# flanggut/smvs

Hardware: NVIDIA H100
Metric: Gauss-Newton Mpix-iters/sec (higher is better)
Workload: dtype f64

## Files before the change

smvs_b200/csrc/api.cu:

```cuda
#include <algorithm>
#include <atomic>
#include <cmath>
#include <cstring>
#include <dlfcn.h>

#include "common.cuh"

namespace smvsb {
void fill_basis_table (std::vector<double>& tab, int ps, int step);
void device_set_scale (smvsb_ctx* c, uint8_t const* img_dev, int w, int h,
    int scale, float* tmp_a, float* tmp_b, int mode, float* out_dev);
void device_shading_inputs (smvsb_ctx* c, uint8_t const* img_dev, int w, int h,
    float* shading_dev, float* shading_grad_dev);
void device_set_scale_float (smvsb_ctx* c, float const* img_dev, int w, int h,
    int scale, float* tmp_a, float* tmp_b, float* out_dev);
void device_set_scale_rgb (smvsb_ctx* c, float const* img_dev, int w, int h,
    int scale, float* tmp_a, float* tmp_b, int mode, float* out_dev,
    float* blur_out);
void device_bilateral_filter (smvsb_ctx* c, float const* ci_dev, int w, int h,
    int channels, float const* dm_dev, int dm_w, int dm_h, float sigma,
    int kernel_size, float* out_dev);
float host_expf_like_glibc (float x);
void device_byte_to_float (smvsb_ctx* c, uint8_t const* img_dev, size_t n,
    float* out_dev);
// ... 176 lines not shown
                    V[i * N + q] = sn * vp + cs * vq;
                }
            }
        if (off < 1e-15)
            break;
    }
    double sinv[16];
    for (int j = 0; j < N; ++j)
    {
        double n = 0.0;
        for (int i = 0; i < N; ++i) n += U[i * N + j] * U[i * N + j];
        n = std::sqrt(n);
        for (int i = 0; i < N; ++i)
            U[i * N + j] = (n > 0.0 ? U[i * N + j] / n : 0.0);
        sinv[j] = (n >= -1e-12 && n <= 1e-12) ? 0.0 : 1.0 / n;
    }
    for (int i = 0; i < N; ++i)
        for (int j = 0; j < N; ++j)
        {
            double s = 0.0;
            for (int k = 0; k < N; ++k)
                s += V[i * N + k] * sinv[k] * U[j * N + k];
            Ainv[i * N + j] = s;
        }
}

void
ensure_system_buffers (smvsb_ctx* c)
{
    size_t const np = c->n_patches, nn = c->n_nodes;
    c->patch_H.reserve(np * 256);
    c->patch_g.reserve(np * 16);
    c->patch_proc.reserve(np);
    c->H.reserve(nn * 144);
    c->P.reserve(nn * 16);
    c->g.reserve(nn * 4);
    c->x.reserve(nn * 4);
    c->light.reserve(16);
}

void
set_active (smvsb_ctx* c, uint8_t const* active_nodes)
{
    if (active_nodes != nullptr)
        upload(c, c->active, active_nodes, c->n_nodes);
    else
    {
        c->active.reserve(c->n_nodes);
        CUDA_CHECK(cudaMemcpyAsync(c->active.p, c->node_valid.p, c->n_nodes,
            cudaMemcpyDeviceToDevice, c->stream));
    }
}

void
construct (smvsb_ctx* c, double const* light16, double reg, double light_reg)
{
    require(c->have_views && c->have_surface, SMVSB_ERR_STATE,
        "smvsb_set_views and smvsb_set_surface must precede construct");
    if (light16 != nullptr)
    {
        require(c->have_shading, SMVSB_ERR_STATE,
            "lighting given but the main view has no shading image");
        upload(c, c->light, light16, 16);
    }
    ensure_system_buffers(c);
    smvsb::launch_construct(c, light16 != nullptr, reg, light_reg);
// ... 1557 lines not shown
```

smvs_b200/csrc/common.cuh:

```cuda
#ifndef SMVSB_COMMON_CUH
#define SMVSB_COMMON_CUH

#include <cuda_runtime.h>

#include <atomic>
#include <cstdint>
#include <cstdio>
#include <string>
#include <vector>

#include "../../include/smvs_b200.h"

#define SMVSB_MAX_SUBS 32
#define SMVSB_NB_STRIDE 8
#define SMVSB_NUM_EVENTS 6

#define CUDA_CHECK(call)                                                     \
    do {                                                                     \
        cudaError_t e__ = (call);                                            \
        if (e__ != cudaSuccess)                                              \
            throw smvsb::Error(SMVSB_ERR_CUDA, std::string(#call) + ": "     \
                + cudaGetErrorString(e__));                                  \
    } while (0)

// ... 83 lines not shown
    smvsb::DevBuf<float> main_grad, main_shading, main_shading_grad;
    bool have_shading = false;
    smvsb::SubViewDev subs[SMVSB_MAX_SUBS];
    smvsb::DevBuf<float const*> sub_ptrs;
    smvsb::DevBuf<int> sub_dims;
    smvsb::DevBuf<double> Mt;
    smvsb::DevBuf<uint8_t> stage_u8;
    smvsb::DevBuf<uint8_t> stage_u8b;
    smvsb::DevBuf<float> stage_a, stage_b;
    smvsb::DevBuf<float> view_in, view_texels, view_out;

    bool have_surface = false;
    int scale = 0, ps = 0, sampling = 0, npos = 0;
    int npx = 0, npy = 0, start_x = 0, start_y = 0;
    int n_nodes = 0, n_patches = 0;
    smvsb::DevBuf<double> nodes;
    smvsb::DevBuf<uint8_t> node_valid, patch_valid, vis_ids;
    smvsb::DevBuf<uint32_t> vis_off;
    smvsb::DevBuf<uint8_t> active, active_new;
    smvsb::DevBuf<double> basis_s, basis_f;
    std::vector<uint8_t> h_node_valid, h_patch_valid;

    smvsb::DevBuf<float> init_depth;
    smvsb::DevBuf<double> nodes_tmp;
    smvsb::DevBuf<uint8_t> node_valid_tmp;
    smvsb::DevBuf<uint8_t> u8_main;
    smvsb::DevBuf<uint8_t> u8_subs[SMVSB_MAX_SUBS];
    smvsb::DevBuf<float> guide;

    bool have_system = false;
    smvsb::DevBuf<double> patch_H;
    smvsb::DevBuf<double> patch_g;
    smvsb::DevBuf<uint8_t> patch_proc;
    smvsb::DevBuf<double> H;
    smvsb::DevBuf<double> P;
    smvsb::DevBuf<double> g;
    smvsb::DevBuf<double> light;

    smvsb::DevBuf<double> x, r, d, d2, z, Ad;
    size_t x_count = 0;
    smvsb::DevBuf<double> cg_partials;
    smvsb::DevBuf<uint16_t> cg_rowmask;
    smvsb::DevBuf<uint32_t> cg_row_list, cg_block_rows;
    smvsb::DevBuf<unsigned long long> cg_counts;
    uint64_t cg_blocks = 0, cg_rows = 0;
    double* h_scalars = nullptr;
    smvsb::DevBuf<unsigned int> cg_sync;
    smvsb::DevBuf<double> cg_result;

    smvsb::DevBuf<double> patch_shift;
    smvsb::DevBuf<double> upd_partials, upd_result;
    smvsb::DevBuf<unsigned long long> counters;

    smvsb::DevBuf<unsigned int> zbuf, vis_mask;
    smvsb::DevBuf<unsigned long long> zoff;
    smvsb::DevBuf<float> sgm_depth;
    bool have_color = false;
    smvsb::DevBuf<float> color_main;
    smvsb::DevBuf<float> color_subs[SMVSB_MAX_SUBS];
    smvsb::DevBuf<float const*> color_ptrs;
    smvsb::DevBuf<short4> rim_lists;
    int rim_ps = 0;
    int rim_off[9] = {};
    smvsb::DevBuf<uint32_t> vis_counts;

    smvsb::DevBuf<double> light_partials;
// ... 87 lines not shown
```

smvs_b200/csrc/gn_construct.cu:

```cuda
#include "gn_math.cuh"
#include "patch_eval.cuh"

namespace smvsb {

namespace {

constexpr int K1_THREADS = 128;
constexpr int AS_STRIDE = 27;

__host__ __device__ inline void
hermite (double t, double* b0, double* b1, double* b2)
{
    double const t2 = t * t, t3 = t2 * t;
    b0[0] = 2 * t3 - 3 * t2 + 1;
    b0[1] = -2 * t3 + 3 * t2;
    b0[2] = t3 - 2 * t2 + t;
    b0[3] = t3 - t2;
    b1[0] = 6 * t2 - 6 * t;
    b1[1] = -6 * t2 + 6 * t;
    b1[2] = 3 * t2 - 4 * t + 1;
    b1[3] = 3 * t2 - 2 * t;
    b2[0] = 12 * t - 6;
    b2[1] = -12 * t + 6;
    b2[2] = 6 * t - 4;
    b2[3] = 6 * t - 2;
}

}

void
fill_basis_table (std::vector<double>& tab, int ps, int step)
{
    int const npos = ps / step;
    tab.assign(3 * npos * 4, 0.0);
    for (int a = 0; a < npos; ++a)
    {
        double b0[4], b1[4], b2[4];
        hermite((a * step + 0.5) / ps, b0, b1, b2);
        for (int i = 0; i < 4; ++i)
        {
            tab[(0 * npos + a) * 4 + i] = b0[i];
// ... 9 lines not shown
    float const* __restrict__ hess, float* __restrict__ texels, int n)
{
    int i = blockIdx.x * blockDim.x + threadIdx.x;
    if (i >= n)
        return;
    float4 a, b;
    a.x = grad[2 * i]; a.y = grad[2 * i + 1];
    a.z = hess[3 * i]; a.w = hess[3 * i + 1];
    b.x = hess[3 * i + 2]; b.y = 0.f; b.z = 0.f; b.w = 0.f;
    reinterpret_cast<float4*>(texels)[2 * i] = a;
    reinterpret_cast<float4*>(texels)[2 * i + 1] = b;
}

void
launch_pack_subview (smvsb_ctx* c, float const* grad, float const* hess,
    float* texels, int w, int h)
{
    int const n = w * h;
    pack_subview_kernel<<<(n + 255) / 256, 256, 0, c->stream>>>(grad, hess,
        texels, n);
    smvsb::count_launches(c, 1);
    CUDA_CHECK(cudaGetLastError());
}


struct ConstructArgs
{
    SurfaceDev s;
    double regularization;
    double light_surf_regularization;
    double const* light;
    double* patch_H;
    double* patch_g;
    uint8_t* patch_proc;
};

template <int S, int MINB = 4>
__global__ void __launch_bounds__(K1_THREADS, MINB)
gn_patch_kernel (ConstructArgs const args)
{
    constexpr int SPC = (S < K1_THREADS) ? S : K1_THREADS;
    constexpr int CHUNKS = S / SPC;
    constexpr int PPB = (S >= 16) ? K1_THREADS / SPC : 8;
    constexpr int GSZ = (S >= 16) ? 16 : S;
    constexpr int GPP = (S >= 16) ? SPC / 16 : 1;
    SurfaceDev const& sf = args.s;

    __shared__ double s_theta[PPB][16];
    __shared__ double s_coef[PPB][16];
    __shared__ double s_as[K1_THREADS * AS_STRIDE];
    __shared__ double s_basis[3 * 16 * 4];
    __shared__ double s_part[(GPP > 1) ? K1_THREADS * 17 : 1];
    __shared__ int s_proc[PPB];

    int const tid = threadIdx.x;
    int const npos = sf.npos;

    for (int i = tid; i < 3 * npos * 4; i += K1_THREADS)
        s_basis[i] = sf.basis_s[i];

    if (tid < PPB)
    {
        int const patch = blockIdx.x * PPB + tid;
        int proc = 0;
        if (patch < sf.n_patches && sf.patch_valid[patch])
        {
            int const idx = patch % sf.npx, idy = patch / sf.npx;
            int const n0 = idy * (sf.npx + 1) + idx;
            proc = sf.active[n0] | sf.active[n0 + 1]
                | sf.active[n0 + sf.npx + 1] | sf.active[n0 + sf.npx + 2];
            proc = proc != 0;
        }
        s_proc[tid] = proc;
        if (patch < sf.n_patches)
            args.patch_proc[patch] = static_cast<uint8_t>(proc);
    }
    if (tid < PPB * 16)
    {
        int const pl = tid / 16, col = tid % 16;
        int const patch = blockIdx.x * PPB + pl;
        double v = 0.0;
        if (patch < sf.n_patches)
        {
            int const idx = patch % sf.npx, idy = patch / sf.npx;
            int const node = (idy + ((col >> 3) & 1)) * (sf.npx + 1)
                + idx + ((col >> 2) & 1);
            v = sf.nodes[node * 4 + (col & 3)];
        }
        s_theta[pl][col] = v;
    }
    __syncthreads();

    if (tid < PPB * 16)
    {
        int const pl = tid / 16, r = tid % 16;
        xd sum(0.0);
#pragma unroll
        for (int k = 0; k < 16; ++k)
        {
            double const xv = s_theta[pl][(k & 3) * 4 + (k >> 2)];
            sum += xd(c_hermite[r * 16 + k]) * xd(xv);
        }
        s_coef[pl][(r & 3) * 4 + (r >> 2)] = sum.v;
    }
    __syncthreads();

    int const q = tid / 16;
    int const row = tid % 16;
    int const pl2 = q / GPP;
    int const patch2 = blockIdx.x * PPB + pl2;
    bool const proc2 = s_proc[pl2] != 0;
    double hrow[16];
    double grow = 0.0;
#pragma unroll
    for (int i = 0; i < 16; ++i) hrow[i] = 0.0;

    for (int chunk = 0; chunk < CHUNKS; ++chunk)
    {
    if (tid < PPB * SPC)
    {
        int const pl = tid / SPC;
        int const s = chunk * SPC + tid % SPC;
        int const patch = blockIdx.x * PPB + pl;
        double A[21], b[6];
#pragma unroll
        for (int i = 0; i < 21; ++i) A[i] = 0.0;
#pragma unroll
        for (int i = 0; i < 6; ++i) b[i] = 0.0;

        if (s_proc[pl])
        {
            int const ix = s % npos, iy = s / npos;

            double w, wx, wy, wxy, wxx, wyy;
            {
                double const* cf = s_coef[pl];
                xd const inv_size(1.0 / static_cast<double>(sf.ps));
                xd const sx = (xd(static_cast<double>(ix * sf.sampling))
                    + xd(0.5)) * inv_size;
                xd const sy = (xd(static_cast<double>(iy * sf.sampling))
                    + xd(0.5)) * inv_size;
                xd ex[4], ey[4];
                ex[0] = xd(1.0); ex[1] = sx; ex[2] = sx * sx; ex[3] = ex[2] * sx;
                ey[0] = xd(1.0); ey[1] = sy; ey[2] = sy * sy; ey[3] = ey[2] * sy;
                xd f(0.0), fx(0.0), fy(0.0), fxy(0.0), fxx(0.0), fyy(0.0);
#pragma unroll
                for (int i = 0; i < 4; ++i)
#pragma unroll
                    for (int j = 0; j < 4; ++j)
                        f += xd(cf[i * 4 + j]) * ex[i] * ey[j];
#pragma unroll
                for (int i = 1; i < 4; ++i)
#pragma unroll
                    for (int j = 0; j < 4; ++j)
                        fx += xd(cf[i * 4 + j]) * xd(double(i)) * ex[i - 1]
                            * ey[j];
#pragma unroll
                for (int i = 2; i < 4; ++i)
#pragma unroll
                    for (int j = 0; j < 4; ++j)
                        fxx += xd(cf[i * 4 + j]) * xd(double(i))
                            * xd(double(i - 1)) * ex[i - 2] * ey[j];
#pragma unroll
                for (int i = 0; i < 4; ++i)
#pragma unroll
                    for (int j = 1; j < 4; ++j)
                        fy += xd(cf[i * 4 + j]) * ex[i] * xd(double(j))
                            * ey[j - 1];
#pragma unroll
                for (int i = 0; i < 4; ++i)
#pragma unroll
                    for (int j = 2; j < 4; ++j)
                        fyy += xd(cf[i * 4 + j]) * ex[i] * xd(double(j))
                            * xd(double(j - 1)) * ey[j - 2];
#pragma unroll
                for (int i = 1; i < 4; ++i)
#pragma unroll
                    for (int j = 1; j < 4; ++j)
                        fxy += xd(cf[i * 4 + j]) * xd(double(i)) * ex[i - 1]
                            * xd(double(j)) * ey[j - 1];
                xd const inv_size2(1.0 / static_cast<double>(sf.ps * sf.ps));
                w = f.v;
                wx = (fx * inv_size).v;
                wy = (fy * inv_size).v;
                wxy = (fxy * inv_size2).v;
                wxx = (fxx * inv_size2).v;
                wyy = (fyy * inv_size2).v;
            }

            int const idx = patch % sf.npx, idy = patch / sf.npx;
            int const px = sf.start_x + idx * sf.ps + ix * sf.sampling;
            int const py = sf.start_y + idy * sf.ps + iy * sf.sampling;
            size_t const pix = static_cast<size_t>(py) * sf.w + px;
            float2 const gm = __ldg(
                reinterpret_cast<float2 const*>(sf.main_grad) + pix);
            double const gmx = gm.x, gmy = gm.y;

            uint32_t const v0 = sf.vis_off[patch];
            int const n = static_cast<int>(sf.vis_off[patch + 1] - v0);
            NbRow rows[SMVSB_MAX_SUBS];
            for (int j = 0; j < n; ++j)
            {
                int const sub = sf.vis_ids[v0 + j];
                rows[j] = neighbour_row(sf.Mt + sub * 12, sf.sub_texels[sub],
                    sf.sub_dims[2 * sub], sf.sub_dims[2 * sub + 1],
                    px + 0.5, py + 0.5, w, wx, wy);
            }

            for (int j = 0; j < n; ++j)
            {
                NbRow const rj = rows[j];
                double const dx_ = rj.jgx - gmx, dy_ = rj.jgy - gmy;
                add_photo_row<1>(A, b, rj.ax, rj.be, dx_,
                    1.0 / (fabs(dx_) + SMVSB_R_FACTOR));
                add_photo_row<2>(A, b, rj.ay, rj.be, dy_,
                    1.0 / (fabs(dy_) + SMVSB_R_FACTOR));
                for (int j2 = j + 1; j2 < n; ++j2)
                {
                    NbRow const r2 = rows[j2];
                    double const sx_ = rj.jgx - r2.jgx;
                    double const sy_ = rj.jgy - r2.jgy;
                    double const be = rj.be - r2.be;
                    add_photo_row<1>(A, b, rj.ax - r2.ax, be, sx_,
                        1.0 / (fabs(sx_) + SMVSB_R_FACTOR));
                    add_photo_row<2>(A, b, rj.ay - r2.ay, be, sy_,
                        1.0 / (fabs(sy_) + SMVSB_R_FACTOR));
                }
            }

            if (args.regularization > 0.0)
            {
                double const num_diffs = double((n * (n + 1)) / 2);
                double const basic = args.regularization * 0.005
                    / fmax(0.03, fabs(gmx) + fabs(gmy)) * num_diffs;
                double const x = px + 0.5 - static_cast<double>(sf.w) / 2.0;
                double const y = py + 0.5 - static_cast<double>(sf.h) / 2.0;
                SurfGeo geo;
                surface_geometry(x, y, sf.flen, w, wx, wy, wxy, wxx, wyy, geo);

                bool const lit = (args.light != nullptr);
                if (!lit || args.light_surf_regularization > 0.0)
                {
                    double geom_weight = 1.0;
                    if (lit)
                        geom_weight *= args.light_surf_regularization / 100;
#pragma unroll
                    for (int v = 0; v < 6; ++v)
                    {
                        double const wgt = geom_weight
                            / (SMVSB_R_FACTOR + fabs(geo.div[v])) * basic;
                        add_full_row(A, b, geo.C[v], geo.div[v], wgt);
                    }
                }

                if (lit)
                {
                    double L[16];
#pragma unroll
                    for (int l = 0; l < 16; ++l) L[l] = args.light[l];
                    double nrm[3];
                    fill_normal(x, y, sf.inv_flen, w, wx, wy, nrm);
                    double sh[16];
                    sh_evaluate_4_band(nrm, sh);
                    double shading = 0.0;
#pragma unroll
                    for (int l = 0; l < 16; ++l) shading += L[l] * sh[l];
                    float2 const lg = __ldg(reinterpret_cast<float2 const*>(
                        sf.main_shading_grad) + pix);
                    double ligx = lg.x, ligy = lg.y;
                    double const liv = __ldg(sf.main_shading + pix);
                    double const shading_weight = 0.001 * num_diffs
                        / (SMVSB_R_FACTOR + fabs(ligx) + fabs(ligy));
                    bool ok = !(sqrt(ligx * ligx + ligy * ligy) < 1e-10);
                    ok = ok && !(shading * shading < 1e-10
                        || liv * liv < 1e-10);
                    if (ok)
                    {
                        double G[3];
                        sh_light_gradient(nrm, L, G);
                        double const sgx = G[0] * geo.div[0]
                            + G[1] * geo.div[1] + G[2] * geo.div[2];
                        double const sgy = G[0] * geo.div[3]
                            + G[1] * geo.div[4] + G[2] * geo.div[5];
                        double const inv_s = 1.0 / shading;
                        ligx *= 1.0 / liv;
                        ligy *= 1.0 / liv;
                        double const ex = sgx * inv_s - ligx;
                        double const ey = sgy * inv_s - ligy;
                        double cx[6], cy[6];
                        double const inv_s2 = 1.0 / (shading * shading);
#pragma unroll
                        for (int k = 0; k < 6; ++k)
                        {
                            double const sd = (k < 3) ? G[0] * geo.N[0][k]
                                + G[1] * geo.N[1][k] + G[2] * geo.N[2][k]
                                : 0.0;
                            double const gdx = G[0] * geo.C[0][k]
                                + G[1] * geo.C[1][k] + G[2] * geo.C[2][k];
                            double const gdy = G[0] * geo.C[3][k]
                                + G[1] * geo.C[4][k] + G[2] * geo.C[5][k];
                            cx[k] = (gdx * shading - sgx * sd) * inv_s2;
                            cy[k] = (gdy * shading - sgy * sd) * inv_s2;
                        }
                        add_full_row(A, b, cx, ex, shading_weight
                            / (SMVSB_R_FACTOR + fabs(ex)));
                        add_full_row(A, b, cy, ey, shading_weight
                            / (SMVSB_R_FACTOR + fabs(ey)));
                    }
                }
            }
        }

        double* dst = s_as + tid * AS_STRIDE;
#pragma unroll
        for (int i = 0; i < 21; ++i) dst[i] = A[i];
#pragma unroll
        for (int i = 0; i < 6; ++i) dst[21 + i] = b[i];
    }
    __syncthreads();

    if (proc2)
    {
        int const rbx = ((row >> 2) & 1) + 2 * (row & 1);
        int const rby = ((row >> 3) & 1) + 2 * ((row >> 1) & 1);
        for (int ss = 0; ss < GSZ; ++ss)
        {
            int const sl = (q % GPP) * GSZ + ss;
            int const s = chunk * SPC + sl;
            int const ix = s % npos, iy = s / npos;
            double const* as = s_as + (pl2 * SPC + sl) * AS_STRIDE;
            double const* X0 = s_basis + (0 * npos + ix) * 4;
            double const* X1 = s_basis + (1 * npos + ix) * 4;
            double const* X2 = s_basis + (2 * npos + ix) * 4;
            double const* Y0 = s_basis + (0 * npos + iy) * 4;
            double const* Y1 = s_basis + (1 * npos + iy) * 4;
            double const* Y2 = s_basis + (2 * npos + iy) * 4;

            double Dr[6];
            Dr[0] = X0[rbx] * Y0[rby];
            Dr[1] = X1[rbx] * Y0[rby];
            Dr[2] = X0[rbx] * Y1[rby];
            Dr[3] = X1[rbx] * Y1[rby];
            Dr[4] = X2[rbx] * Y0[rby];
            Dr[5] = X0[rbx] * Y2[rby];

            double E[6];
#pragma unroll
            for (int k = 0; k < 6; ++k)
            {
                double e = 0.0;
#pragma unroll
                for (int l = 0; l < 6; ++l)
                    e += as[(k <= l) ? sym6(k, l) : sym6(l, k)] * Dr[l];
                E[k] = e;
                grow += as[21 + k] * Dr[k];
            }

            double U0[4], U1[4], U2[4];
#pragma unroll
            for (int j = 0; j < 4; ++j)
            {
                U0[j] = E[0] * Y0[j] + E[2] * Y1[j] + E[5] * Y2[j];
                U1[j] = E[1] * Y0[j] + E[3] * Y1[j];
                U2[j] = E[4] * Y0[j];
            }
#pragma unroll
            for (int col = 0; col < 16; ++col)
            {
                int const bx = ((col >> 2) & 1) + 2 * (col & 1);
                int const by = ((col >> 3) & 1) + 2 * ((col >> 1) & 1);
                hrow[col] += X0[bx] * U0[by] + X1[bx] * U1[by]
                    + X2[bx] * U2[by];
            }
        }
    }
    if (CHUNKS > 1)
        __syncthreads();
    }

    if (GPP == 1)
    {
        if (proc2 && patch2 < sf.n_patches)
        {
            double2* dst = reinterpret_cast<double2*>(
                args.patch_H + (static_cast<size_t>(patch2) * 16 + row) * 16);
#pragma unroll
            for (int i = 0; i < 8; ++i)
                dst[i] = make_double2(hrow[2 * i], hrow[2 * i + 1]);
            args.patch_g[static_cast<size_t>(patch2) * 16 + row] = grow;
        }
    }
    else
    {
        double* part = s_part + tid * 17;
#pragma unroll
        for (int i = 0; i < 16; ++i) part[i] = hrow[i];
        part[16] = grow;
        __syncthreads();
        if (tid < PPB * 16)
        {
            int const pl = tid / 16, r = tid % 16;
            int const patch = blockIdx.x * PPB + pl;
            if (s_proc[pl] && patch < sf.n_patches)
            {
                double acc[17];
#pragma unroll
                for (int i = 0; i < 17; ++i) acc[i] = 0.0;
                for (int gq = 0; gq < GPP; ++gq)
                {
                    double const* p = s_part
                        + ((pl * GPP + gq) * 16 + r) * 17;
#pragma unroll
                    for (int i = 0; i < 17; ++i) acc[i] += p[i];
                }
                double* dst = args.patch_H
                    + (static_cast<size_t>(patch) * 16 + r) * 16;
#pragma unroll
                for (int i = 0; i < 16; ++i) dst[i] = acc[i];
                args.patch_g[static_cast<size_t>(patch) * 16 + r] = acc[16];
            }
        }
    }
}


__global__ void
gn_assemble_kernel (SurfaceDev const sf, double const* __restrict__ patch_H,
    double const* __restrict__ patch_g,
    uint8_t const* __restrict__ patch_proc, double* __restrict__ H,
    double* __restrict__ g)
{
    int const gid = blockIdx.x * blockDim.x + threadIdx.x;
    int const node = gid / 36;
    int const rem = gid % 36;
    int const k = rem / 4, rp = rem % 4;
    if (node >= sf.n_nodes)
        return;

    int const ns = sf.npx + 1;
    int const ix = node % ns, iy = node / ns;
    int const dx = k % 3 - 1, dy = k / 3 - 1;
    int const jx = ix + dx, jy = iy + dy;

    double acc[4] = {0.0, 0.0, 0.0, 0.0};
    double gacc = 0.0;
    bool const row_on = sf.node_valid[node] && sf.active[node];
    bool col_on = false;
    if (jx >= 0 && jx <= sf.npx && jy >= 0 && jy <= sf.npy)
    {
        int const nj = jy * ns + jx;
        col_on = sf.node_valid[nj] && sf.active[nj];
    }

    if (row_on)
// ... 40 lines not shown
    if (node >= sf.n_nodes)
        return;
    double A[16], out[16];
    bool const on = sf.node_valid[node] && sf.active[node];
    double const* src = H + (static_cast<size_t>(node) * 9 + 4) * 16;
#pragma unroll
    for (int i = 0; i < 16; ++i) A[i] = on ? src[i] : 0.0;
    if (on)
    {
        bool ok = ldl_inverse4(A, out);
        if (ok)
        {
            bool nan = false;
#pragma unroll
            for (int i = 0; i < 16; ++i) nan = nan || isnan(out[i]);
            ok = !nan;
        }
        if (!ok)
        {
#pragma unroll
            for (int i = 0; i < 16; ++i) out[i] = A[i];
        }
    }
    else
    {
#pragma unroll
        for (int i = 0; i < 16; ++i) out[i] = 0.0;
    }
    double* dst = P + static_cast<size_t>(node) * 16;
#pragma unroll
    for (int i = 0; i < 16; ++i) dst[i] = out[i];
}

void
launch_construct (smvsb_ctx* c, bool use_light, double reg, double light_reg)
{
    ConstructArgs a;
    a.s = surface_args(c);
    a.regularization = reg;
    a.light_surf_regularization = light_reg;
    a.light = use_light ? c->light.p : nullptr;
    a.patch_H = c->patch_H.p;
    a.patch_g = c->patch_g.p;
    a.patch_proc = c->patch_proc.p;

    int const S = c->npos * c->npos;
    auto blocks = [&](int ppb) { return (c->n_patches + ppb - 1) / ppb; };
    switch (S)
    {
    case 1:
        gn_patch_kernel<1><<<blocks(8), K1_THREADS, 0, c->stream>>>(a); break;
    case 4:
        gn_patch_kernel<4><<<blocks(8), K1_THREADS, 0, c->stream>>>(a); break;
    case 16:
    {
        gn_patch_kernel<16><<<blocks(8), K1_THREADS, 0, c->stream>>>(a);
        break;
    }
    case 64:
        gn_patch_kernel<64><<<blocks(2), K1_THREADS, 0, c->stream>>>(a); break;
    case 256:
        gn_patch_kernel<256><<<blocks(1), K1_THREADS, 0, c->stream>>>(a); break;
    default:
        throw Error(SMVSB_ERR_INVALID, "unsupported samples per patch");
    }
    CUDA_CHECK(cudaGetLastError());

    int const n_thr = c->n_nodes * 36;
    gn_assemble_kernel<<<(n_thr + 287) / 288, 288, 0, c->stream>>>(a.s,
        c->patch_H.p, c->patch_g.p, c->patch_proc.p, c->H.p, c->g.p);
    CUDA_CHECK(cudaGetLastError());
    gn_precond_kernel<<<(c->n_nodes + 127) / 128, 128, 0, c->stream>>>(a.s,
        c->H.p, c->P.p);
    CUDA_CHECK(cudaGetLastError());
    smvsb::count_launches(c, 3);
}

}
```

Before: 145.0.

## Compact active patches into a list and specialize patch kernel on lighting

Adds a pre-pass kernel that computes the per-patch process flag and compacts the active patch indices into a list with warp-aggregated atomics. The patch kernel then works only on listed patches, and blocks past the list end exit early. The kernel is also templated on lighting, and for unlit runs with few neighbour views it keeps neighbour rows in shared memory rather than in a local register array. This costs an extra launch, a memset and the atomic compaction, and patch order in the list becomes nondeterministic, though outputs are written by patch index.

Measured after the change: 148.8 (median of 6 runs). +2.6%, better.

```diff
diff --git a/smvs_b200/csrc/api.cu b/smvs_b200/csrc/api.cu
--- a/smvs_b200/csrc/api.cu
+++ b/smvs_b200/csrc/api.cu
@@ -232,6 +232,7 @@
     c->patch_H.reserve(np * 256);
     c->patch_g.reserve(np * 16);
     c->patch_proc.reserve(np);
+    c->patch_list.reserve(np + 1);
     c->H.reserve(nn * 144);
     c->P.reserve(nn * 16);
     c->g.reserve(nn * 4);
diff --git a/smvs_b200/csrc/common.cuh b/smvs_b200/csrc/common.cuh
--- a/smvs_b200/csrc/common.cuh
+++ b/smvs_b200/csrc/common.cuh
@@ -139,6 +139,7 @@
     smvsb::DevBuf<double> patch_H;
     smvsb::DevBuf<double> patch_g;
     smvsb::DevBuf<uint8_t> patch_proc;
+    smvsb::DevBuf<uint32_t> patch_list;
     smvsb::DevBuf<double> H;
     smvsb::DevBuf<double> P;
     smvsb::DevBuf<double> g;
diff --git a/smvs_b200/csrc/gn_construct.cu b/smvs_b200/csrc/gn_construct.cu
--- a/smvs_b200/csrc/gn_construct.cu
+++ b/smvs_b200/csrc/gn_construct.cu
@@ -6,7 +6,20 @@
 namespace {
 
 constexpr int K1_THREADS = 128;
-constexpr int AS_STRIDE = 27;
+constexpr int K1_MIN_BLOCKS = 4;
+constexpr int K1_NB = 6;
+
+__host__ __device__ constexpr int
+as_stride (bool srows)
+{
+    return ((srows && 5 * K1_NB > 27) ? 5 * K1_NB : 27) | 1;
+}
+
+__host__ __device__ constexpr int
+k1_patches_per_block (int S)
+{
+    return (S >= 16) ? K1_THREADS / ((S < K1_THREADS) ? S : K1_THREADS) : 8;
+}
 
 __host__ __device__ inline void
 hermite (double t, double* b0, double* b1, double* b2)
@@ -82,18 +95,49 @@
     double const* light;
     double* patch_H;
     double* patch_g;
-    uint8_t* patch_proc;
+    uint32_t const* patch_list;
 };
 
-template <int S, int MINB = 4>
-__global__ void __launch_bounds__(K1_THREADS, MINB)
+__global__ void __launch_bounds__(256)
+gn_patch_list_kernel (SurfaceDev const sf, uint8_t* __restrict__ patch_proc,
+    uint32_t* __restrict__ list)
+{
+    int const patch = blockIdx.x * blockDim.x + threadIdx.x;
+    bool proc = false;
+    if (patch < sf.n_patches)
+    {
+        if (sf.patch_valid[patch])
+        {
+            int const idx = patch % sf.npx, idy = patch / sf.npx;
+            int const n0 = idy * (sf.npx + 1) + idx;
+            proc = (sf.active[n0] | sf.active[n0 + 1]
+                | sf.active[n0 + sf.npx + 1] | sf.active[n0 + sf.npx + 2]) != 0;
+        }
+        patch_proc[patch] = static_cast<uint8_t>(proc);
+    }
+    unsigned int const mask = __ballot_sync(0xffffffffu, proc);
+    if (mask == 0)
+        return;
+    int const lane = threadIdx.x & 31, leader = __ffs(mask) - 1;
+    uint32_t base = 0;
+    if (lane == leader)
+        base = atomicAdd(list, static_cast<uint32_t>(__popc(mask)));
+    base = __shfl_sync(0xffffffffu, base, leader);
+    if (proc)
+        list[1 + base + __popc(mask & ((1u << lane) - 1u))] = patch;
+}
+
+template <int S, bool LIT, bool SROWS>
+__global__ void __launch_bounds__(K1_THREADS, K1_MIN_BLOCKS)
 gn_patch_kernel (ConstructArgs const args)
 {
     constexpr int SPC = (S < K1_THREADS) ? S : K1_THREADS;
     constexpr int CHUNKS = S / SPC;
-    constexpr int PPB = (S >= 16) ? K1_THREADS / SPC : 8;
+    constexpr int PPB = k1_patches_per_block(S);
     constexpr int GSZ = (S >= 16) ? 16 : S;
     constexpr int GPP = (S >= 16) ? SPC / 16 : 1;
+    constexpr int AS_STRIDE = as_stride(SROWS);
+    static_assert(!SROWS || (!LIT && S < 64), "shared rows: unlit, S < 64");
     SurfaceDev const& sf = args.s;
 
     __shared__ double s_theta[PPB][16];
@@ -101,36 +145,31 @@
     __shared__ double s_as[K1_THREADS * AS_STRIDE];
     __shared__ double s_basis[3 * 16 * 4];
     __shared__ double s_part[(GPP > 1) ? K1_THREADS * 17 : 1];
-    __shared__ int s_proc[PPB];
+    __shared__ int s_patch[PPB];
 
     int const tid = threadIdx.x;
     int const npos = sf.npos;
 
+    int const n_list = static_cast<int>(args.patch_list[0]);
+    if (static_cast<int>(blockIdx.x) * PPB >= n_list)
+        return;
+
     for (int i = tid; i < 3 * npos * 4; i += K1_THREADS)
         s_basis[i] = sf.basis_s[i];
-
     if (tid < PPB)
     {
-        int const patch = blockIdx.x * PPB + tid;
-        int proc = 0;
-        if (patch < sf.n_patches && sf.patch_valid[patch])
-        {
-            int const idx = patch % sf.npx, idy = patch / sf.npx;
-            int const n0 = idy * (sf.npx + 1) + idx;
-            proc = sf.active[n0] | sf.active[n0 + 1]
-                | sf.active[n0 + sf.npx + 1] | sf.active[n0 + sf.npx + 2];
-            proc = proc != 0;
-        }
-        s_proc[tid] = proc;
-        if (patch < sf.n_patches)
-            args.patch_proc[patch] = static_cast<uint8_t>(proc);
-    }
+        int const k = blockIdx.x * PPB + tid;
+        s_patch[tid] = (k < n_list) ? static_cast<int>(args.patch_list[1 + k])
+            : -1;
+    }
+    __syncthreads();
+
     if (tid < PPB * 16)
     {
         int const pl = tid / 16, col = tid % 16;
-        int const patch = blockIdx.x * PPB + pl;
+        int const patch = s_patch[pl];
         double v = 0.0;
-        if (patch < sf.n_patches)
+        if (patch >= 0)
         {
             int const idx = patch % sf.npx, idy = patch / sf.npx;
             int const node = (idy + ((col >> 3) & 1)) * (sf.npx + 1)
@@ -158,8 +197,8 @@
     int const q = tid / 16;
     int const row = tid % 16;
     int const pl2 = q / GPP;
-    int const patch2 = blockIdx.x * PPB + pl2;
-    bool const proc2 = s_proc[pl2] != 0;
+    int const patch2 = s_patch[pl2];
+    bool const proc2 = patch2 >= 0;
     double hrow[16];
     double grow = 0.0;
 #pragma unroll
@@ -171,14 +210,14 @@
     {
         int const pl = tid / SPC;
         int const s = chunk * SPC + tid % SPC;
-        int const patch = blockIdx.x * PPB + pl;
+        int const patch = s_patch[pl];
         double A[21], b[6];
 #pragma unroll
         for (int i = 0; i < 21; ++i) A[i] = 0.0;
 #pragma unroll
         for (int i = 0; i < 6; ++i) b[i] = 0.0;
 
-        if (s_proc[pl])
+        if (patch >= 0)
         {
             int const ix = s % npos, iy = s / npos;
 
@@ -248,18 +287,38 @@
 
             uint32_t const v0 = sf.vis_off[patch];
             int const n = static_cast<int>(sf.vis_off[patch + 1] - v0);
-            NbRow rows[SMVSB_MAX_SUBS];
+            NbRow lrows[SROWS ? 1 : SMVSB_MAX_SUBS];
+            double* const srows = s_as + tid * AS_STRIDE;
+            auto put_row = [&](int j, NbRow const& r) {
+                if constexpr (SROWS)
+                {
+                    double* const d = srows + 5 * j;
+                    d[0] = r.jgx; d[1] = r.jgy; d[2] = r.ax; d[3] = r.ay;
+                    d[4] = r.be;
+                }
+                else
+                    lrows[j] = r;
+            };
+            auto get_row = [&](int j) {
+                if constexpr (SROWS)
+                {
+                    double const* const d = srows + 5 * j;
+                    return NbRow{d[0], d[1], d[2], d[3], d[4]};
+                }
+                else
+                    return lrows[j];
+            };
             for (int j = 0; j < n; ++j)
             {
                 int const sub = sf.vis_ids[v0 + j];
-                rows[j] = neighbour_row(sf.Mt + sub * 12, sf.sub_texels[sub],
+                put_row(j, neighbour_row(sf.Mt + sub * 12, sf.sub_texels[sub],
                     sf.sub_dims[2 * sub], sf.sub_dims[2 * sub + 1],
-                    px + 0.5, py + 0.5, w, wx, wy);
+                    px + 0.5, py + 0.5, w, wx, wy));
             }
 
             for (int j = 0; j < n; ++j)
             {
-                NbRow const rj = rows[j];
+                NbRow const rj = get_row(j);
                 double const dx_ = rj.jgx - gmx, dy_ = rj.jgy - gmy;
                 add_photo_row<1>(A, b, rj.ax, rj.be, dx_,
                     1.0 / (fabs(dx_) + SMVSB_R_FACTOR));
@@ -267,7 +326,7 @@
                     1.0 / (fabs(dy_) + SMVSB_R_FACTOR));
                 for (int j2 = j + 1; j2 < n; ++j2)
                 {
-                    NbRow const r2 = rows[j2];
+                    NbRow const r2 = get_row(j2);
                     double const sx_ = rj.jgx - r2.jgx;
                     double const sy_ = rj.jgy - r2.jgy;
                     double const be = rj.be - r2.be;
@@ -288,11 +347,10 @@
                 SurfGeo geo;
                 surface_geometry(x, y, sf.flen, w, wx, wy, wxy, wxx, wyy, geo);
 
-                bool const lit = (args.light != nullptr);
-                if (!lit || args.light_surf_regularization > 0.0)
+                if (!LIT || args.light_surf_regularization > 0.0)
                 {
                     double geom_weight = 1.0;
-                    if (lit)
+                    if (LIT)
                         geom_weight *= args.light_surf_regularization / 100;
 #pragma unroll
                     for (int v = 0; v < 6; ++v)
@@ -303,7 +361,7 @@
                     }
                 }
 
-                if (lit)
+                if constexpr (LIT)
                 {
                     double L[16];
 #pragma unroll
@@ -430,7 +488,7 @@
 
     if (GPP == 1)
     {
-        if (proc2 && patch2 < sf.n_patches)
+        if (proc2)
         {
             double2* dst = reinterpret_cast<double2*>(
                 args.patch_H + (static_cast<size_t>(patch2) * 16 + row) * 16);
@@ -450,8 +508,8 @@
         if (tid < PPB * 16)
         {
             int const pl = tid / 16, r = tid % 16;
-            int const patch = blockIdx.x * PPB + pl;
-            if (s_proc[pl] && patch < sf.n_patches)
+            int const patch = s_patch[pl];
+            if (patch >= 0)
             {
                 double acc[17];
 #pragma unroll
@@ -576,6 +634,19 @@
     for (int i = 0; i < 16; ++i) dst[i] = out[i];
 }
 
+template <int S>
+void
+launch_patch_kernel (smvsb_ctx* c, ConstructArgs const& a, bool lit)
+{
+    constexpr int PPB = k1_patches_per_block(S);
+    auto kernel = lit ? gn_patch_kernel<S, true, false>
+        : gn_patch_kernel<S, false, false>;
+    if constexpr (S < 64)
+        if (!lit && c->n_sub <= K1_NB)
+            kernel = gn_patch_kernel<S, false, true>;
+    kernel<<<(c->n_patches + PPB - 1) / PPB, K1_THREADS, 0, c->stream>>>(a);
+}
+
 void
 launch_construct (smvsb_ctx* c, bool use_light, double reg, double light_reg)
 {
@@ -586,25 +657,21 @@
     a.light = use_light ? c->light.p : nullptr;
     a.patch_H = c->patch_H.p;
     a.patch_g = c->patch_g.p;
-    a.patch_proc = c->patch_proc.p;
+    a.patch_list = c->patch_list.p;
+
+    CUDA_CHECK(cudaMemsetAsync(c->patch_list.p, 0, sizeof(uint32_t), c->stream));
+    gn_patch_list_kernel<<<(c->n_patches + 255) / 256, 256, 0, c->stream>>>(
+        a.s, c->patch_proc.p, c->patch_list.p);
+    CUDA_CHECK(cudaGetLastError());
 
     int const S = c->npos * c->npos;
-    auto blocks = [&](int ppb) { return (c->n_patches + ppb - 1) / ppb; };
     switch (S)
     {
-    case 1:
-        gn_patch_kernel<1><<<blocks(8), K1_THREADS, 0, c->stream>>>(a); break;
-    case 4:
-        gn_patch_kernel<4><<<blocks(8), K1_THREADS, 0, c->stream>>>(a); break;
-    case 16:
-    {
-        gn_patch_kernel<16><<<blocks(8), K1_THREADS, 0, c->stream>>>(a);
-        break;
-    }
-    case 64:
-        gn_patch_kernel<64><<<blocks(2), K1_THREADS, 0, c->stream>>>(a); break;
-    case 256:
-        gn_patch_kernel<256><<<blocks(1), K1_THREADS, 0, c->stream>>>(a); break;
+    case 1: launch_patch_kernel<1>(c, a, use_light); break;
+    case 4: launch_patch_kernel<4>(c, a, use_light); break;
+    case 16: launch_patch_kernel<16>(c, a, use_light); break;
+    case 64: launch_patch_kernel<64>(c, a, use_light); break;
+    case 256: launch_patch_kernel<256>(c, a, use_light); break;
     default:
         throw Error(SMVSB_ERR_INVALID, "unsupported samples per patch");
     }
@@ -617,7 +684,7 @@
     gn_precond_kernel<<<(c->n_nodes + 127) / 128, 128, 0, c->stream>>>(a.s,
         c->H.p, c->P.p);
     CUDA_CHECK(cudaGetLastError());
-    smvsb::count_launches(c, 3);
-}
-
-}
+    smvsb::count_launches(c, 4);
+}
+
+}
```

## Parallelize neighbour-row evaluation across block threads via shared memory staging

Applied to the files above, without the earlier changes.

The per-sample serial loop that computed neighbour rows for every visible sub-view is replaced by a block-wide work list: each thread computes one (sample, neighbour) row and stores it in a shared-memory region, with a fallback recompute for neighbours beyond a cap. Shared memory becomes dynamic and aliased between row staging, the A/b scratch, and chunk partials, and the regularization terms now accumulate straight into shared scratch. The lighting flag becomes a template parameter. This targets load imbalance and register pressure from the per-thread rows array, at the cost of extra barriers and larger shared memory that may reduce occupancy.

New measurement: 145.8 before, 147.6 after, median of 6. 1.2% higher.

```diff
diff --git a/smvs_b200/csrc/gn_construct.cu b/smvs_b200/csrc/gn_construct.cu
--- a/smvs_b200/csrc/gn_construct.cu
+++ b/smvs_b200/csrc/gn_construct.cu
@@ -7,6 +7,19 @@
 
 constexpr int K1_THREADS = 128;
 constexpr int AS_STRIDE = 27;
+constexpr int PART_STRIDE = 17;
+constexpr int NB_FIELDS = 5;
+constexpr int NB_CAP = 8;
+constexpr int K1_REGION = NB_FIELDS * NB_CAP * K1_THREADS;
+static_assert(NB_FIELDS * NB_CAP >= AS_STRIDE
+    && NB_FIELDS * NB_CAP >= PART_STRIDE, "K1 region too small");
+
+__host__ __device__ constexpr int
+k1_smem_doubles (int S)
+{
+    return K1_REGION + (S > K1_THREADS ? K1_THREADS * PART_STRIDE : 0)
+        + 3 * K1_THREADS;
+}
 
 __host__ __device__ inline void
 hermite (double t, double* b0, double* b1, double* b2)
@@ -85,7 +98,7 @@
     uint8_t* patch_proc;
 };
 
-template <int S, int MINB = 4>
+template <int S, bool LIT, int MINB = 4>
 __global__ void __launch_bounds__(K1_THREADS, MINB)
 gn_patch_kernel (ConstructArgs const args)
 {
@@ -96,12 +109,17 @@
     constexpr int GPP = (S >= 16) ? SPC / 16 : 1;
     SurfaceDev const& sf = args.s;
 
+    extern __shared__ double k1_smem[];
+    double* const s_rows = k1_smem;
+    double* const s_as = k1_smem;
+    double* const s_part = (CHUNKS > 1) ? k1_smem + K1_REGION : k1_smem;
+    double* const s_w = k1_smem + k1_smem_doubles(S) - 3 * K1_THREADS;
     __shared__ double s_theta[PPB][16];
     __shared__ double s_coef[PPB][16];
-    __shared__ double s_as[K1_THREADS * AS_STRIDE];
     __shared__ double s_basis[3 * 16 * 4];
-    __shared__ double s_part[(GPP > 1) ? K1_THREADS * 17 : 1];
     __shared__ int s_proc[PPB];
+    __shared__ int s_nvis[PPB];
+    __shared__ int s_roff[PPB + 1];
 
     int const tid = threadIdx.x;
     int const npos = sf.npos;
@@ -122,6 +140,8 @@
             proc = proc != 0;
         }
         s_proc[tid] = proc;
+        s_nvis[tid] = proc ? static_cast<int>(sf.vis_off[patch + 1]
+            - sf.vis_off[patch]) : 0;
         if (patch < sf.n_patches)
             args.patch_proc[patch] = static_cast<uint8_t>(proc);
     }
@@ -152,6 +172,16 @@
             sum += xd(c_hermite[r * 16 + k]) * xd(xv);
         }
         s_coef[pl][(r & 3) * 4 + (r >> 2)] = sum.v;
+    }
+    if (tid == 0)
+    {
+        int o = 0;
+        for (int p = 0; p < PPB; ++p)
+        {
+            s_roff[p] = o;
+            o += SPC * min(s_nvis[p], NB_CAP);
+        }
+        s_roff[PPB] = o;
     }
     __syncthreads();
 
@@ -160,215 +190,274 @@
     int const pl2 = q / GPP;
     int const patch2 = blockIdx.x * PPB + pl2;
     bool const proc2 = s_proc[pl2] != 0;
-    double hrow[16];
-    double grow = 0.0;
-#pragma unroll
-    for (int i = 0; i < 16; ++i) hrow[i] = 0.0;
 
     for (int chunk = 0; chunk < CHUNKS; ++chunk)
     {
-    if (tid < PPB * SPC)
-    {
-        int const pl = tid / SPC;
-        int const s = chunk * SPC + tid % SPC;
-        int const patch = blockIdx.x * PPB + pl;
-        double A[21], b[6];
-#pragma unroll
-        for (int i = 0; i < 21; ++i) A[i] = 0.0;
-#pragma unroll
-        for (int i = 0; i < 6; ++i) b[i] = 0.0;
-
-        if (s_proc[pl])
-        {
-            int const ix = s % npos, iy = s / npos;
-
-            double w, wx, wy, wxy, wxx, wyy;
-            {
-                double const* cf = s_coef[pl];
-                xd const inv_size(1.0 / static_cast<double>(sf.ps));
-                xd const sx = (xd(static_cast<double>(ix * sf.sampling))
-                    + xd(0.5)) * inv_size;
-                xd const sy = (xd(static_cast<double>(iy * sf.sampling))
-                    + xd(0.5)) * inv_size;
-                xd ex[4], ey[4];
-                ex[0] = xd(1.0); ex[1] = sx; ex[2] = sx * sx; ex[3] = ex[2] * sx;
-                ey[0] = xd(1.0); ey[1] = sy; ey[2] = sy * sy; ey[3] = ey[2] * sy;
-                xd f(0.0), fx(0.0), fy(0.0), fxy(0.0), fxx(0.0), fyy(0.0);
-#pragma unroll
-                for (int i = 0; i < 4; ++i)
-#pragma unroll
-                    for (int j = 0; j < 4; ++j)
-                        f += xd(cf[i * 4 + j]) * ex[i] * ey[j];
-#pragma unroll
-                for (int i = 1; i < 4; ++i)
-#pragma unroll
-                    for (int j = 0; j < 4; ++j)
-                        fx += xd(cf[i * 4 + j]) * xd(double(i)) * ex[i - 1]
-                            * ey[j];
-#pragma unroll
-                for (int i = 2; i < 4; ++i)
-#pragma unroll
-                    for (int j = 0; j < 4; ++j)
-                        fxx += xd(cf[i * 4 + j]) * xd(double(i))
-                            * xd(double(i - 1)) * ex[i - 2] * ey[j];
-#pragma unroll
-                for (int i = 0; i < 4; ++i)
-#pragma unroll
-                    for (int j = 1; j < 4; ++j)
-                        fy += xd(cf[i * 4 + j]) * ex[i] * xd(double(j))
-                            * ey[j - 1];
-#pragma unroll
-                for (int i = 0; i < 4; ++i)
-#pragma unroll
-                    for (int j = 2; j < 4; ++j)
-                        fyy += xd(cf[i * 4 + j]) * ex[i] * xd(double(j))
-                            * xd(double(j - 1)) * ey[j - 2];
-#pragma unroll
-                for (int i = 1; i < 4; ++i)
-#pragma unroll
-                    for (int j = 1; j < 4; ++j)
-                        fxy += xd(cf[i * 4 + j]) * xd(double(i)) * ex[i - 1]
-                            * xd(double(j)) * ey[j - 1];
-                xd const inv_size2(1.0 / static_cast<double>(sf.ps * sf.ps));
-                w = f.v;
-                wx = (fx * inv_size).v;
-                wy = (fy * inv_size).v;
-                wxy = (fxy * inv_size2).v;
-                wxx = (fxx * inv_size2).v;
-                wyy = (fyy * inv_size2).v;
-            }
-
-            int const idx = patch % sf.npx, idy = patch / sf.npx;
-            int const px = sf.start_x + idx * sf.ps + ix * sf.sampling;
-            int const py = sf.start_y + idy * sf.ps + iy * sf.sampling;
-            size_t const pix = static_cast<size_t>(py) * sf.w + px;
-            float2 const gm = __ldg(
-                reinterpret_cast<float2 const*>(sf.main_grad) + pix);
-            double const gmx = gm.x, gmy = gm.y;
-
-            uint32_t const v0 = sf.vis_off[patch];
-            int const n = static_cast<int>(sf.vis_off[patch + 1] - v0);
-            NbRow rows[SMVSB_MAX_SUBS];
-            for (int j = 0; j < n; ++j)
+    int const pl = tid / SPC;
+    int const s = chunk * SPC + tid % SPC;
+    int const patch = blockIdx.x * PPB + pl;
+    bool const smp = tid < PPB * SPC && s_proc[pl];
+    int const ix = s % npos, iy = s / npos;
+    int px = 0, py = 0;
+    double w = 0.0, wx = 0.0, wy = 0.0, wxy = 0.0, wxx = 0.0, wyy = 0.0;
+    if (smp)
+    {
+        double const* cf = s_coef[pl];
+        xd const inv_size(1.0 / static_cast<double>(sf.ps));
+        xd const sx = (xd(static_cast<double>(ix * sf.sampling))
+            + xd(0.5)) * inv_size;
+        xd const sy = (xd(static_cast<double>(iy * sf.sampling))
+            + xd(0.5)) * inv_size;
+        xd ex[4], ey[4];
+        ex[0] = xd(1.0); ex[1] = sx; ex[2] = sx * sx; ex[3] = ex[2] * sx;
+        ey[0] = xd(1.0); ey[1] = sy; ey[2] = sy * sy; ey[3] = ey[2] * sy;
+        xd f(0.0), fx(0.0), fy(0.0), fxy(0.0), fxx(0.0), fyy(0.0);
+#pragma unroll
+        for (int i = 0; i < 4; ++i)
+#pragma unroll
+            for (int j = 0; j < 4; ++j)
+                f += xd(cf[i * 4 + j]) * ex[i] * ey[j];
+#pragma unroll
+        for (int i = 1; i < 4; ++i)
+#pragma unroll
+            for (int j = 0; j < 4; ++j)
+                fx += xd(cf[i * 4 + j]) * xd(double(i)) * ex[i - 1]
+                    * ey[j];
+#pragma unroll
+        for (int i = 2; i < 4; ++i)
+#pragma unroll
+            for (int j = 0; j < 4; ++j)
+                fxx += xd(cf[i * 4 + j]) * xd(double(i))
+                    * xd(double(i - 1)) * ex[i - 2] * ey[j];
+#pragma unroll
+        for (int i = 0; i < 4; ++i)
+#pragma unroll
+            for (int j = 1; j < 4; ++j)
+                fy += xd(cf[i * 4 + j]) * ex[i] * xd(double(j))
+                    * ey[j - 1];
+#pragma unroll
+        for (int i = 0; i < 4; ++i)
+#pragma unroll
+            for (int j = 2; j < 4; ++j)
+                fyy += xd(cf[i * 4 + j]) * ex[i] * xd(double(j))
+                    * xd(double(j - 1)) * ey[j - 2];
+#pragma unroll
+        for (int i = 1; i < 4; ++i)
+#pragma unroll
+            for (int j = 1; j < 4; ++j)
+                fxy += xd(cf[i * 4 + j]) * xd(double(i)) * ex[i - 1]
+                    * xd(double(j)) * ey[j - 1];
+        xd const inv_size2(1.0 / static_cast<double>(sf.ps * sf.ps));
+        w = f.v;
+        wx = (fx * inv_size).v;
+        wy = (fy * inv_size).v;
+        wxy = (fxy * inv_size2).v;
+        wxx = (fxx * inv_size2).v;
+        wyy = (fyy * inv_size2).v;
+
+        px = sf.start_x + (patch % sf.npx) * sf.ps + ix * sf.sampling;
+        py = sf.start_y + (patch / sf.npx) * sf.ps + iy * sf.sampling;
+        s_w[tid] = w;
+        s_w[K1_THREADS + tid] = wx;
+        s_w[2 * K1_THREADS + tid] = wy;
+    }
+    __syncthreads();
+
+    for (int i = tid; i < s_roff[PPB]; i += K1_THREADS)
+    {
+        int p = 0;
+#pragma unroll
+        for (int k = 1; k < PPB; ++k)
+            p += (i >= s_roff[k]);
+        int const k = i - s_roff[p];
+        int const j = k / SPC, sl = k % SPC;
+        int const ptc = blockIdx.x * PPB + p;
+        int const sr = chunk * SPC + sl;
+        int const rpx = sf.start_x + (ptc % sf.npx) * sf.ps
+            + (sr % npos) * sf.sampling;
+        int const rpy = sf.start_y + (ptc / sf.npx) * sf.ps
+            + (sr / npos) * sf.sampling;
+        int const slot = p * SPC + sl;
+        int const sub = sf.vis_ids[sf.vis_off[ptc] + j];
+        NbRow const r = neighbour_row(sf.Mt + sub * 12, sf.sub_texels[sub],
+            sf.sub_dims[2 * sub], sf.sub_dims[2 * sub + 1], rpx + 0.5,
+            rpy + 0.5, s_w[slot], s_w[K1_THREADS + slot],
+            s_w[2 * K1_THREADS + slot]);
+        double* dst = s_rows + j * NB_FIELDS * K1_THREADS + slot;
+        dst[0 * K1_THREADS] = r.jgx;
+        dst[1 * K1_THREADS] = r.jgy;
+        dst[2 * K1_THREADS] = r.ax;
+        dst[3 * K1_THREADS] = r.ay;
+        dst[4 * K1_THREADS] = r.be;
+    }
+    __syncthreads();
+
+    double A[21], b[6];
+#pragma unroll
+    for (int i = 0; i < 21; ++i) A[i] = 0.0;
+#pragma unroll
+    for (int i = 0; i < 6; ++i) b[i] = 0.0;
+    int const n = smp ? s_nvis[pl] : 0;
+    size_t const pix = static_cast<size_t>(py) * sf.w + px;
+    double gmx = 0.0, gmy = 0.0;
+    if (smp)
+    {
+        float2 const gm = __ldg(
+            reinterpret_cast<float2 const*>(sf.main_grad) + pix);
+        gmx = gm.x;
+        gmy = gm.y;
+        uint32_t const v0 = sf.vis_off[patch];
+        auto row_of = [&](int j) {
+            NbRow r;
+            if (j < NB_CAP)
+            {
+                double const* src = s_rows + j * NB_FIELDS * K1_THREADS + tid;
+                r.jgx = src[0 * K1_THREADS];
+                r.jgy = src[1 * K1_THREADS];
+                r.ax = src[2 * K1_THREADS];
+                r.ay = src[3 * K1_THREADS];
+                r.be = src[4 * K1_THREADS];
+            }
+            else
             {
                 int const sub = sf.vis_ids[v0 + j];
-                rows[j] = neighbour_row(sf.Mt + sub * 12, sf.sub_texels[sub],
+                r = neighbour_row(sf.Mt + sub * 12, sf.sub_texels[sub],
                     sf.sub_dims[2 * sub], sf.sub_dims[2 * sub + 1],
                     px + 0.5, py + 0.5, w, wx, wy);
             }
-
-            for (int j = 0; j < n; ++j)
-            {
-                NbRow const rj = rows[j];
-                double const dx_ = rj.jgx - gmx, dy_ = rj.jgy - gmy;
-                add_photo_row<1>(A, b, rj.ax, rj.be, dx_,
-                    1.0 / (fabs(dx_) + SMVSB_R_FACTOR));
-                add_photo_row<2>(A, b, rj.ay, rj.be, dy_,
-                    1.0 / (fabs(dy_) + SMVSB_R_FACTOR));
-                for (int j2 = j + 1; j2 < n; ++j2)
+            return r;
+        };
+
+        for (int j = 0; j < n; ++j)
+        {
+            NbRow const rj = row_of(j);
+            double const dx_ = rj.jgx - gmx, dy_ = rj.jgy - gmy;
+            add_photo_row<1>(A, b, rj.ax, rj.be, dx_,
+                1.0 / (fabs(dx_) + SMVSB_R_FACTOR));
+            add_photo_row<2>(A, b, rj.ay, rj.be, dy_,
+                1.0 / (fabs(dy_) + SMVSB_R_FACTOR));
+            for (int j2 = j + 1; j2 < n; ++j2)
+            {
+                NbRow const r2 = row_of(j2);
+                double const sx_ = rj.jgx - r2.jgx;
+                double const sy_ = rj.jgy - r2.jgy;
+                double const be = rj.be - r2.be;
+                add_photo_row<1>(A, b, rj.ax - r2.ax, be, sx_,
+                    1.0 / (fabs(sx_) + SMVSB_R_FACTOR));
+                add_photo_row<2>(A, b, rj.ay - r2.ay, be, sy_,
+                    1.0 / (fabs(sy_) + SMVSB_R_FACTOR));
+            }
+        }
+    }
+    __syncthreads();
+
+    double* const as = s_as + tid * AS_STRIDE;
+    if (tid < PPB * SPC)
+    {
+#pragma unroll
+        for (int i = 0; i < 21; ++i) as[i] = A[i];
+#pragma unroll
+        for (int i = 0; i < 6; ++i) as[21 + i] = b[i];
+    }
+
+    if (smp && args.regularization > 0.0)
+    {
+        double const num_diffs = double((n * (n + 1)) / 2);
+        double const basic = args.regularization * 0.005
+            / fmax(0.03, fabs(gmx) + fabs(gmy)) * num_diffs;
+        double const x = px + 0.5 - static_cast<double>(sf.w) / 2.0;
+        double const y = py + 0.5 - static_cast<double>(sf.h) / 2.0;
+        SurfGeo geo;
+        surface_geometry(x, y, sf.flen, w, wx, wy, wxy, wxx, wyy, geo);
+
+        bool const lit = LIT;
+        if (!lit || args.light_surf_regularization > 0.0)
+        {
+            double geom_weight = 1.0;
+            if (lit)
+                geom_weight *= args.light_surf_regularization / 100;
+#pragma unroll
+            for (int v = 0; v < 6; ++v)
+            {
+                double const wgt = geom_weight
+                    / (SMVSB_R_FACTOR + fabs(geo.div[v])) * basic;
+                add_full_row(as, as + 21, geo.C[v], geo.div[v], wgt);
+            }
+        }
+
+        if (lit)
+        {
+            double L[16];
+#pragma unroll
+            for (int l = 0; l < 16; ++l) L[l] = args.light[l];
+            double nrm[3];
+            fill_normal(x, y, sf.inv_flen, w, wx, wy, nrm);
+            double sh[16];
+            sh_evaluate_4_band(nrm, sh);
+            double shading = 0.0;
+#pragma unroll
+            for (int l = 0; l < 16; ++l) shading += L[l] * sh[l];
+            float2 const lg = __ldg(reinterpret_cast<float2 const*>(
+                sf.main_shading_grad) + pix);
+            double ligx = lg.x, ligy = lg.y;
+            double const liv = __ldg(sf.main_shading + pix);
+            double const shading_weight = 0.001 * num_diffs
+                / (SMVSB_R_FACTOR + fabs(ligx) + fabs(ligy));
+            bool ok = !(sqrt(ligx * ligx + ligy * ligy) < 1e-10);
+            ok = ok && !(shading * shading < 1e-10
+                || liv * liv < 1e-10);
+            if (ok)
+            {
+                double G[3];
+                sh_light_gradient(nrm, L, G);
+                double const sgx = G[0] * geo.div[0]
+                    + G[1] * geo.div[1] + G[2] * geo.div[2];
+                double const sgy = G[0] * geo.div[3]
+                    + G[1] * geo.div[4] + G[2] * geo.div[5];
+                double const inv_s = 1.0 / shading;
+                ligx *= 1.0 / liv;
+                ligy *= 1.0 / liv;
+                double const ex = sgx * inv_s - ligx;
+                double const ey = sgy * inv_s - ligy;
+                double cx[6], cy[6];
+                double const inv_s2 = 1.0 / (shading * shading);
+#pragma unroll
+                for (int k = 0; k < 6; ++k)
                 {
-                    NbRow const r2 = rows[j2];
-                    double const sx_ = rj.jgx - r2.jgx;
-                    double const sy_ = rj.jgy - r2.jgy;
-                    double const be = rj.be - r2.be;
-                    add_photo_row<1>(A, b, rj.ax - r2.ax, be, sx_,
-                        1.0 / (fabs(sx_) + SMVSB_R_FACTOR));
-                    add_photo_row<2>(A, b, rj.ay - r2.ay, be, sy_,
-                        1.0 / (fabs(sy_) + SMVSB_R_FACTOR));
+                    double const sd = (k < 3) ? G[0] * geo.N[0][k]
+                        + G[1] * geo.N[1][k] + G[2] * geo.N[2][k]
+                        : 0.0;
+                    double const gdx = G[0] * geo.C[0][k]
+                        + G[1] * geo.C[1][k] + G[2] * geo.C[2][k];
+                    double const gdy = G[0] * geo.C[3][k]
+                        + G[1] * geo.C[4][k] + G[2] * geo.C[5][k];
+                    cx[k] = (gdx * shading - sgx * sd) * inv_s2;
+                    cy[k] = (gdy * shading - sgy * sd) * inv_s2;
                 }
-            }
-
-            if (args.regularization > 0.0)
-            {
-                double const num_diffs = double((n * (n + 1)) / 2);
-                double const basic = args.regularization * 0.005
-                    / fmax(0.03, fabs(gmx) + fabs(gmy)) * num_diffs;
-                double const x = px + 0.5 - static_cast<double>(sf.w) / 2.0;
-                double const y = py + 0.5 - static_cast<double>(sf.h) / 2.0;
-                SurfGeo geo;
-                surface_geometry(x, y, sf.flen, w, wx, wy, wxy, wxx, wyy, geo);
-
-                bool const lit = (args.light != nullptr);
-                if (!lit || args.light_surf_regularization > 0.0)
-                {
-                    double geom_weight = 1.0;
-                    if (lit)
-                        geom_weight *= args.light_surf_regularization / 100;
-#pragma unroll
-                    for (int v = 0; v < 6; ++v)
-                    {
-                        double const wgt = geom_weight
-                            / (SMVSB_R_FACTOR + fabs(geo.div[v])) * basic;
-                        add_full_row(A, b, geo.C[v], geo.div[v], wgt);
-                    }
-                }
-
-                if (lit)
-                {
-                    double L[16];
-#pragma unroll
-                    for (int l = 0; l < 16; ++l) L[l] = args.light[l];
-                    double nrm[3];
-                    fill_normal(x, y, sf.inv_flen, w, wx, wy, nrm);
-                    double sh[16];
-                    sh_evaluate_4_band(nrm, sh);
-                    double shading = 0.0;
-#pragma unroll
-                    for (int l = 0; l < 16; ++l) shading += L[l] * sh[l];
-                    float2 const lg = __ldg(reinterpret_cast<float2 const*>(
-                        sf.main_shading_grad) + pix);
-                    double ligx = lg.x, ligy = lg.y;
-                    double const liv = __ldg(sf.main_shading + pix);
-                    double const shading_weight = 0.001 * num_diffs
-                        / (SMVSB_R_FACTOR + fabs(ligx) + fabs(ligy));
-                    bool ok = !(sqrt(ligx * ligx + ligy * ligy) < 1e-10);
-                    ok = ok && !(shading * shading < 1e-10
-                        || liv * liv < 1e-10);
-                    if (ok)
-                    {
-                        double G[3];
-                        sh_light_gradient(nrm, L, G);
-                        double const sgx = G[0] * geo.div[0]
-                            + G[1] * geo.div[1] + G[2] * geo.div[2];
-                        double const sgy = G[0] * geo.div[3]
-                            + G[1] * geo.div[4] + G[2] * geo.div[5];
-                        double const inv_s = 1.0 / shading;
-                        ligx *= 1.0 / liv;
-                        ligy *= 1.0 / liv;
-                        double const ex = sgx * inv_s - ligx;
-                        double const ey = sgy * inv_s - ligy;
-                        double cx[6], cy[6];
-                        double const inv_s2 = 1.0 / (shading * shading);
-#pragma unroll
-                        for (int k = 0; k < 6; ++k)
-                        {
-                            double const sd = (k < 3) ? G[0] * geo.N[0][k]
-                                + G[1] * geo.N[1][k] + G[2] * geo.N[2][k]
-                                : 0.0;
-                            double const gdx = G[0] * geo.C[0][k]
-                                + G[1] * geo.C[1][k] + G[2] * geo.C[2][k];
-                            double const gdy = G[0] * geo.C[3][k]
-                                + G[1] * geo.C[4][k] + G[2] * geo.C[5][k];
-                            cx[k] = (gdx * shading - sgx * sd) * inv_s2;
-                            cy[k] = (gdy * shading - sgy * sd) * inv_s2;
-                        }
-                        add_full_row(A, b, cx, ex, shading_weight
-                            / (SMVSB_R_FACTOR + fabs(ex)));
-                        add_full_row(A, b, cy, ey, shading_weight
-                            / (SMVSB_R_FACTOR + fabs(ey)));
-                    }
-                }
-            }
-        }
-
-        double* dst = s_as + tid * AS_STRIDE;
-#pragma unroll
-        for (int i = 0; i < 21; ++i) dst[i] = A[i];
-#pragma unroll
-        for (int i = 0; i < 6; ++i) dst[21 + i] = b[i];
-    }
+                add_full_row(as, as + 21, cx, ex, shading_weight
+                    / (SMVSB_R_FACTOR + fabs(ex)));
+                add_full_row(as, as + 21, cy, ey, shading_weight
+                    / (SMVSB_R_FACTOR + fabs(ey)));
+            }
+        }
+    }
+
     __syncthreads();
 
+    double hrow[16];
+    double grow;
+    if (chunk == 0)
+    {
+#pragma unroll
+        for (int i = 0; i < 16; ++i) hrow[i] = 0.0;
+        grow = 0.0;
+    }
+    else
+    {
+#pragma unroll
+        for (int i = 0; i < 16; ++i) hrow[i] = s_part[tid * PART_STRIDE + i];
+        grow = s_part[tid * PART_STRIDE + 16];
+    }
     if (proc2)
     {
         int const rbx = ((row >> 2) & 1) + 2 * (row & 1);
@@ -424,8 +513,13 @@
             }
         }
     }
-    if (CHUNKS > 1)
+    if (chunk + 1 < CHUNKS)
+    {
+#pragma unroll
+        for (int i = 0; i < 16; ++i) s_part[tid * PART_STRIDE + i] = hrow[i];
+        s_part[tid * PART_STRIDE + 16] = grow;
         __syncthreads();
+        continue;
     }
 
     if (GPP == 1)
@@ -442,7 +536,9 @@
     }
     else
     {
-        double* part = s_part + tid * 17;
+        if (CHUNKS == 1)
+            __syncthreads();
+        double* part = s_part + tid * PART_STRIDE;
 #pragma unroll
         for (int i = 0; i < 16; ++i) part[i] = hrow[i];
         part[16] = grow;
@@ -459,7 +555,7 @@
                 for (int gq = 0; gq < GPP; ++gq)
                 {
                     double const* p = s_part
-                        + ((pl * GPP + gq) * 16 + r) * 17;
+                        + ((pl * GPP + gq) * 16 + r) * PART_STRIDE;
 #pragma unroll
                     for (int i = 0; i < 17; ++i) acc[i] += p[i];
                 }
@@ -470,6 +566,7 @@
                 args.patch_g[static_cast<size_t>(patch) * 16 + r] = acc[16];
             }
         }
+    }
     }
 }
 
@@ -590,21 +687,32 @@
 
     int const S = c->npos * c->npos;
     auto blocks = [&](int ppb) { return (c->n_patches + ppb - 1) / ppb; };
+    auto launch = [&](auto unlit, auto lit, int ppb) {
+        auto const kernel = (a.light != nullptr) ? lit : unlit;
+        size_t const smem = sizeof(double) * k1_smem_doubles(S);
+        if (smem > 48 * 1024)
+            CUDA_CHECK(cudaFuncSetAttribute(kernel,
+                cudaFuncAttributeMaxDynamicSharedMemorySize,
+                static_cast<int>(smem)));
+        kernel<<<blocks(ppb), K1_THREADS, smem, c->stream>>>(a);
+    };
     switch (S)
     {
     case 1:
-        gn_patch_kernel<1><<<blocks(8), K1_THREADS, 0, c->stream>>>(a); break;
+        launch(gn_patch_kernel<1, false>, gn_patch_kernel<1, true>, 8);
+        break;
     case 4:
-        gn_patch_kernel<4><<<blocks(8), K1_THREADS, 0, c->stream>>>(a); break;
+        launch(gn_patch_kernel<4, false>, gn_patch_kernel<4, true>, 8);
+        break;
     case 16:
-    {
-        gn_patch_kernel<16><<<blocks(8), K1_THREADS, 0, c->stream>>>(a);
+        launch(gn_patch_kernel<16, false>, gn_patch_kernel<16, true>, 8);
         break;
-    }
     case 64:
-        gn_patch_kernel<64><<<blocks(2), K1_THREADS, 0, c->stream>>>(a); break;
+        launch(gn_patch_kernel<64, false>, gn_patch_kernel<64, true>, 2);
+        break;
     case 256:
-        gn_patch_kernel<256><<<blocks(1), K1_THREADS, 0, c->stream>>>(a); break;
+        launch(gn_patch_kernel<256, false>, gn_patch_kernel<256, true>, 1);
+        break;
     default:
         throw Error(SMVSB_ERR_INVALID, "unsupported samples per patch");
     }
```
